# ImIntheMiddle/VATL4Pose-WACV2024

Hardware: AMD Instinct MI355X
Metric: frames/sec pose-infer+uncertainty, 256x192 17-kp (higher is better)
Workload: dtype f32; 1 GPU; SimpleBaseline-R50 256x192 inference + decode + local-peak + THC-L1, 1024-frame synthetic video per GPU; frames_per_gpu=1024, batch=1024, tracks=4, parallelism=frame-sharded x1

## Files before the change

include/vatl_hip.h:

```cpp
#ifndef VATL_HIP_H
#define VATL_HIP_H

#include <stdint.h>

#ifdef __cplusplus
extern "C" {
#endif

#define VATL_VERSION 100
#define VATL_EINVAL  (-1)
#define VATL_ELAUNCH (-2)

int         vatl_version(void);
const char* vatl_last_error(void);

int vatl_flop_meter_begin(void);
int vatl_flop_meter_end(double* direct_flops, double* winograd_flops, int64_t* direct_launches, int64_t* winograd_launches);
#define VATL_ROUTE_NAMES "igemm,igemm_bnbwd,igemm_dma,persistent_1x1,streamk,rows_1x1,bottleneck_chain,stem_pool,halo_3x3," \
                         "winograd,winograd_2h,winograd_bnbwd,winograd_persist,winograd_c32,wgrad,winograd_wgrad,winograd_wgrad_2h," \
                         "winograd_wgrad_table,winograd_f4,winograd_f4_bnbwd,gemm1x1_ring,winograd_deconv43,winograd_s2_43,stem_pool_w1d," \
                         "chain_proj,chain_step"
int vatl_flop_meter_routes(int64_t* counts, int n);


int vatl_nchw_to_nhwc(const float* src, float* dst, int N, int C, int H, int W, int Cpad, void* stream);
int vatl_nhwc_to_nchw(const float* src, float* dst, int N, int C, int H, int W, void* stream);

int vatl_pack_conv_weight(const float* w_oihw, float* w_packed, int Cout, int Cin, int R, int S,
                          int CoutPad, int Spad, int CinPad, void* stream);
int vatl_pack_deconv4x4s2_weight(const float* w_iohw, float* w_packed, int Cin, int Cout, int CoutPad, void* stream);
int64_t vatl_stem_pool_weight_floats(void);
int vatl_pack_stem_pool_weight(const float* w_oihw, float* packed, void* stream);
int vatl_stem_pool_supported(int H, int W);
int vatl_stem7x7s2_pool_fwd(const float* x_nchw, const float* w_packed, const float* scale, const float* bias, float* y_nhwc,
                            int N, int H, int W, void* stream);
int64_t vatl_stem_pool_w1d_weight_floats(void);
int vatl_pack_stem_pool_w1d_weight(const float* w_oihw, float* packed, void* stream);
int vatl_stem_pool_w1d_supported(int H, int W);
int vatl_stem7x7s2_pool_w1d_fwd(const float* x_nchw, const float* w_packed, const float* scale, const float* bias, float* y_nhwc,
                                int N, int H, int W, void* stream);
int64_t vatl_stem3_weight_floats(void);
int vatl_pack_stem3_weight(const float* w_oihw, float* packed, void* stream);
int vatl_stem3x3s2_fwd(const float* x_nchw, const float* w_packed, const float* scale, const float* bias, float* y_nhwc,
                       int N, int H, int W, void* stream);

// ... 19 lines not shown
                                 int Cin, int Cout, int relu, void* stream);
int64_t vatl_winograd_f4_stats_row_blocks(int64_t N, int H, int W);
int vatl_conv3x3_winograd_f4_fwd_stats(const float* x, const float* u, float* y, double* stats, int64_t* row_blocks_used, int N, int H, int W, int Cin, int Cout,
                                       void* stream);
int vatl_conv3x3_winograd_f4_fwd_bnbwd(const float* x, const float* u, const float* residual, float* y, int N, int H, int W, int Cin, int Cout, const float* bn_z,
                                       const float* bn_mask_y, const float* bn_scale, const float* bn_bias, const float* bn_mean, const float* bn_invstd,
                                       double* stats, int64_t* row_blocks_used, void* stream);

int vatl_conv1x1_rows_supported(int K1, int K2, int N, int64_t M);
int vatl_conv1x1_rows_fwd(const float* a, const float* x2, const float* w, const float* scale, const float* bias, const float* residual, float* y,
                          int64_t M, int K1, int K2, int N, int relu, void* stream);

int vatl_bottleneck_chain_supported(int Cmid, int Cout, int Cnext, int64_t M);
int vatl_bottleneck_chain_fwd(const float* a, const float* w3, const float* scale3, const float* bias3, const float* skip, float* t,
                              const float* w1, const float* scale1, const float* bias1, float* y1, int64_t M, int Cmid, int Cout,
                              int Cnext, void* stream);

int vatl_chain_proj_supported(int Cmid, int Cout, int Cnext, int64_t M);
int vatl_chain_proj_fwd(const float* a, const float* x2, const float* w, const float* scale, const float* bias, float* t, const float* w1,
                        const float* scale1, const float* bias1, float* y1, int64_t M, int Cmid, int Cout, int Cnext, int relu, void* stream);
int vatl_chain_step_supported(int Cmid, int Cout, int Cnext, int64_t M);
int vatl_chain_step_fwd(const float* a, const float* w3, const float* scale3, const float* bias3, const float* skip, float* t, const float* w1,
                        const float* scale1, const float* bias1, float* y1, int64_t M, int Cmid, int Cout, int Cnext, void* stream);

int vatl_tune_set(int knob, int value);
int vatl_set_splitk_workspace(float* workspace, int64_t floats);
int vatl_set_splitk_workspace_thread(float* workspace, int64_t floats);
int64_t vatl_streamk_workspace_bytes(void);
int vatl_set_streamk_workspace_thread(void* workspace, int64_t bytes);
int vatl_conv_cout_pad(int Cout);
int vatl_conv2d_fwd(const float* x, const float* w, const float* scale, const float* bias, const float* residual,
                    float* y, int N, int H, int W, int Cin, int Cout, int CoutPad, int R, int S, int stride, int pad,
                    int relu, int out_nchw, void* stream);

int vatl_deconv4x4s2_fwd(const float* x, const float* w, const float* scale, const float* bias, float* y,
                         int N, int H, int W, int Cin, int Cout, int CoutPad, int relu, void* stream);

int vatl_maxpool3x3s2_fwd(const float* x, float* y, int N, int H, int W, int C, void* stream);
int vatl_gap_fwd(const float* x, float* y, int N, int HW, int C, void* stream);

int vatl_pixelshuffle2_fwd(const float* x, float* y, int N, int H, int W, int C, void* stream);
int vatl_se_scale_add_relu(const float* x, const float* gate, const float* residual, float* y, int N, int HW, int C, void* stream);
int vatl_fuse_upsample_add(const float* base, const float* z0, int shift0, const float* z1, int shift1, const float* z2, int shift2,
                           float* y, int N, int H, int W, int C, int relu, void* stream);
int vatl_upsample_nearest_bwd(const float* dy, const float* yact_or_null, float* dz, int N, int H, int W, int C, int shift, void* stream);
int vatl_gap_bwd(const float* dy, float* dx, int N, int HW, int C, void* stream);
// ... 215 lines not shown
```

vatl4pose-wacv2024_amd/alphapose/models/hip_engine.py:

```python
from __future__ import annotations

import time
import weakref

import torch
import torch.nn as nn

import vatl_hip as vh

MAX_CHUNK = 1024



WINOGRAD = True
ROWS_GEMM = True
ROWS_GEMM_K = (128, 256)
WINO_C32 = True
WINO_F4 = True
DECONV_43 = True
S2_43 = True


class _Conv:
    __slots__ = ("w", "u", "u32", "u4", "us2", "wsrc", "wino", "c32", "f4", "s2", "scale", "bias", "cout", "r", "s", "stride", "pad")
# ... 66 lines not shown
        return vh.deconv4x4s2_fwd(x, self.w, self.scale, self.bias, self.cout, relu)


def _d(p):
    return None if p is None else p.detach()


FUSE_PROJ = True


class _BottleneckPlan:
    def __init__(self, blk):
        self.c1 = _Conv(blk.conv1, blk.bn1)
        self.c2 = _Conv(blk.conv2, blk.bn2)
        self.c3 = _Conv(blk.conv3, blk.bn3)
        self.proj = _Conv(blk.downsample[0], blk.downsample[1]) if blk.downsample is not None else None
        self.dual = None
        if (FUSE_PROJ and self.proj is not None and type(self) is _BottleneckPlan and self.proj.r == 1 and self.c3.cout >= 128
                and blk.conv3.in_channels % 32 == 0 and blk.downsample[0].in_channels % 32 == 0):
            w, b = vh.pack_conv1x1_dual_weight(blk.conv3.weight.detach(), self.c3.scale, self.c3.bias, blk.downsample[0].weight.detach(),
                                               self.proj.scale, self.proj.bias)
            self.dual = (w, b, self.proj.stride)

    def __call__(self, x, out=None, y1=None, nxt=None):
        y = y1 if y1 is not None else self.c1(x, relu=True)
        y = self.c2(y, relu=True)
        return self.tail(y, x, out=out, nxt=nxt)

    def tail(self, y, x, out=None, nxt=None):
        if self.dual is not None:
            if (ROWS_GEMM and self.dual[2] == 1 and y.shape[-1] == 64 and x.shape[-1] == 64 and not vh.latency_mode()
                    and vh.conv1x1_rows_supported(64, 64, self.c3.cout, y.shape[0] * y.shape[1] * y.shape[2])):
                if nxt is not None and FUSE_CHAIN_PROJ and vh.chain_proj_supported(64, self.c3.cout, nxt[0].shape[0], y.shape[0] * y.shape[1] * y.shape[2]):
                    return vh.conv1x1_rows_fwd(y, self.dual[0], None, self.dual[1], self.c3.cout, True, x2=x, out=out, next_conv1=nxt)
                t = vh.conv1x1_rows_fwd(y, self.dual[0], None, self.dual[1], self.c3.cout, True, x2=x, out=out)
            else:
                t = vh.conv1x1_dual_fwd(y, x, self.dual[0], self.dual[1], self.c3.cout, self.dual[2], True, out=out)
        else:
            skip = x if self.proj is None else self.proj(x, relu=False)
            t = self.c3(y, relu=True, residual=skip, out=out)
        return t if nxt is None else (t, None)


FUSE_CHAIN = True
FUSE_CHAIN_PROJ = True
FUSE_CHAIN_STEP = True


def _conv1_of(nxt, cout):
    if (type(nxt) is _BottleneckPlan and (nxt.c1.r, nxt.c1.stride, nxt.c1.pad) == (1, 1, 0) and nxt.c1.scale is not None and nxt.c1.cout == cout
            and not vh.latency_mode()):
        return nxt.c1.w, nxt.c1.scale, nxt.c1.bias
    return None


def _run_blocks(blocks, x, out=None):
    y1 = None
    for k, b in enumerate(blocks):
        last = k == len(blocks) - 1
        o = out if last else None
        if type(b) is not _BottleneckPlan:
            x, y1 = b(x), None
            continue
        nxt = None if last else blocks[k + 1]
        m = x.shape[0] * x.shape[1] * x.shape[2]
        chain = (FUSE_CHAIN and b.proj is None and not vh.latency_mode() and b.c3.scale is not None
                 and vh.bottleneck_chain_supported(b.c3.w.shape[-1], b.c3.cout, 0, m))
        if not chain:
            c1 = _conv1_of(nxt, 64) if b.dual is not None and FUSE_CHAIN_PROJ else None
            x, y1 = b(x, out=o, y1=y1, nxt=c1) if c1 is not None else (b(x, out=o, y1=y1), None)
            continue
        y = b.c2(y1 if y1 is not None else b.c1(x, relu=True), relu=True)
        link, step = _conv1_of(nxt, 64), _conv1_of(nxt, 128) if FUSE_CHAIN_STEP else None
        if link is not None and vh.bottleneck_chain_supported(b.c3.w.shape[-1], b.c3.cout, 64, m):
            x, y1 = vh.bottleneck_chain_fwd(y, b.c3.w, b.c3.scale, b.c3.bias, x, *link, out=o)
        elif step is not None and vh.chain_step_supported(b.c3.w.shape[-1], b.c3.cout, 128, m):
            x, y1 = vh.bottleneck_chain_fwd(y, b.c3.w, b.c3.scale, b.c3.bias, x, out=o, next_stage_conv1=step)
        else:
            x, y1 = vh.bottleneck_chain_fwd(y, b.c3.w, b.c3.scale, b.c3.bias, x, out=o)[0], None
    return x


FUSE_STEM = True
STEM_W1D = True


def _stem_pool_weight(net):
    c = net.conv1
    ok = (FUSE_STEM and tuple(c.weight.shape) == (64, 3, 7, 7) and c.stride == (2, 2) and c.padding == (3, 3) and c.bias is None
          and isinstance(net.maxpool, nn.MaxPool2d) and net.maxpool.kernel_size in (3, (3, 3)) and net.maxpool.stride in (2, (2, 2))
          and net.maxpool.padding in (1, (1, 1)) and not net.maxpool.ceil_mode)
    return vh.pack_stem_pool_weight(c.weight.detach()) if ok else None


class _TrunkPlan:
    def __init__(self, net):
        self.stem = _Conv(net.conv1, net.bn1)
        self.stem_pw = _stem_pool_weight(net)
        self.stem_src, self.stem_u1d = net.conv1.weight.detach(), None
        self.blocks = [_BottleneckPlan(b) for stage in net.stages() for b in stage]
# ... 408 lines not shown
```

vatl4pose-wacv2024_amd/csrc/bottleneck_chain.hip:

```cpp
#include "common.h"
#include "buffer.h"

namespace vatl {

struct ChainParams {
    const float* a;
    const float* w3;
    const float* scale3;
    const float* bias3;
    const float* res;
    float* t;
    const float* w1;
    const float* scale1;
    const float* bias1;
    float* out2;
    int M, N2, relu3;
    int m_tiles;
    unsigned a_bytes, t_bytes, o_bytes, w3_bytes, w1_bytes;
};

constexpr unsigned BOOB = 0xFFFFFFFFu;

constexpr int BT_LDT = 260;
constexpr int BT_AS = 32 * 64;
// ... 137 lines not shown
                    buf_store4(orr, ((unsigned)(mt * 32 + row) * 64u + (unsigned)q4 * 4u) * 4u, o);
                }
            }
        }
        if constexpr (SECOND) asm volatile("s_waitcnt vmcnt(10)" ::: "memory");
        else asm volatile("s_waitcnt vmcnt(8)" ::: "memory");
    }
}


struct FormParams {
    const float* a;
    const float* x2;
    const float* w3;
    const float* scale3;
    const float* bias3;
    const float* res;
    float* t;
    const float* w1;
    const float* scale1;
    const float* bias1;
    float* y;
    int m_tiles, relu3;
    unsigned a_bytes, t_bytes, y_bytes;
};

__device__ __forceinline__ unsigned uadd(unsigned s_part, unsigned v_part) {
#if defined(__HIP_DEVICE_COMPILE__)
    unsigned r;
    asm("v_add_u32 %0, %1, %2" : "=v"(r) : "s"(s_part), "v"(v_part));
    return r;
#else
    return s_part + v_part;
#endif
}

constexpr int CF_TS = 4 * 32 * 64;

template <bool PROJ>
__global__ __launch_bounds__(256, 2) void chain_form_kernel(FormParams p) {
    constexpr int K1 = PROJ ? 128 : 64, G1 = K1 / 8, AS = 32 * K1, N2 = PROJ ? 64 : 128;
    extern __shared__ __attribute__((aligned(16))) float smem[];
    float* As = smem;
    float* Ts = smem + 2 * AS;
    const int tid = threadIdx.x, lane = tid & 63, wave = __builtin_amdgcn_readfirstlane(tid >> 6);
    const int fr = lane & 31, h = lane >> 5;
    const int nblk = gridDim.x;

    const __amdgpu_buffer_rsrc_t ar = buf_rsrc(p.a, p.a_bytes);
    const __amdgpu_buffer_rsrc_t xr = buf_rsrc(PROJ ? p.x2 : p.a, PROJ ? p.a_bytes : 0u);
    const __amdgpu_buffer_rsrc_t w3r = buf_rsrc(p.w3, 256u * K1 * 4u);
    const __amdgpu_buffer_rsrc_t w1r = buf_rsrc(p.w1, (unsigned)N2 * 256u * 4u);
    const __amdgpu_buffer_rsrc_t tr = buf_rsrc(p.t, p.t_bytes);
    const __amdgpu_buffer_rsrc_t rr = buf_rsrc(p.res ? p.res : p.t, p.res ? p.t_bytes : 0u);
    const __amdgpu_buffer_rsrc_t yr = buf_rsrc(p.y, p.y_bytes);

    f32x4 w3f[2][G1];
#pragma unroll
    for (int nb = 0; nb < 2; ++nb)
#pragma unroll
        for (int g = 0; g < G1; ++g) w3f[nb][g] = buf_load4(w3r, (unsigned)(((wave * 64 + nb * 32 + fr) * K1 + 8 * g + 4 * h) * 4));
    float sc3[2], bi3[2];
#pragma unroll
    for (int nb = 0; nb < 2; ++nb) {
        const int n = wave * 64 + nb * 32 + fr;
        sc3[nb] = p.scale3 ? p.scale3[n] : 1.f;
        bi3[nb] = p.bias3 ? p.bias3[n] : 0.f;
    }
    const int l16 = lane & 15, j = lane >> 4;
    const int n1 = PROJ ? wave * 16 + l16 : wave * 32 + fr;
    f32x4 w1f[PROJ ? 16 : 32];
#pragma unroll
    for (int g = 0; g < (PROJ ? 16 : 32); ++g) w1f[g] = buf_load4(w1r, (unsigned)((n1 * 256 + (PROJ ? 16 * g + 4 * j : 8 * g + 4 * h)) * 4));
    const float sc1 = p.scale1 ? p.scale1[n1] : 1.f, bi1 = p.bias1 ? p.bias1[n1] : 0.f;
    const float lo3 = p.relu3 ? 0.f : -INFINITY;

    const int c4 = lane, r0 = wave;
// ... 47 lines not shown
        __builtin_amdgcn_sched_barrier(0);
        const int abase = buf * AS, tqbase = wave * 2048;
#pragma unroll
        for (int nb = 0; nb < 2; ++nb) {
            f32x16 acc;
#pragma unroll
            for (int e = 0; e < 16; ++e) acc[e] = 0.f;
#pragma unroll
            for (int g = 0; g < G1; ++g) {
                const f32x4 af = *reinterpret_cast<const f32x4*>(smem + abase + ax[g & 3] + 32 * (g >> 2));
#pragma unroll
                for (int tt = 0; tt < 4; ++tt) acc = __builtin_amdgcn_mfma_f32_32x32x2f32(af[tt], w3f[nb][g][tt], acc, 0, 0, 0);
            }
            if (!PROJ && nb == 0) asm volatile("s_waitcnt vmcnt(2)" ::: "memory");
#pragma unroll
            for (int e = 0; e < 16; ++e) {
                float* q = smem + tqbase + tq[e & 3] + 64 * ((e & 3) + 8 * (e >> 2)) + 32 * nb;
                const float v = acc[e] * sc3[nb] + bi3[nb];
                *q = fmaxf(v + (PROJ ? 0.f : *q), lo3);
            }
        }
        lds_barrier();
#pragma unroll
        for (int u = 0; u < 8; ++u)
            buf_store4(tr, uadd((unsigned)mt * (32u * 1024u) + (unsigned)(r0 + 4 * u) * 1024u, (unsigned)c4 * 16u),
                       *reinterpret_cast<const f32x4*>(smem + r0 * 64 + tw[u & 1] + 256 * u));
        const unsigned ytile = (unsigned)mt * (32u * N2 * 4u) + (unsigned)wave * (PROJ ? 64u : 128u);
        if constexpr (PROJ) {
            f32x4 acc2[2] = {f32x4{0.f, 0.f, 0.f, 0.f}, f32x4{0.f, 0.f, 0.f, 0.f}};
#pragma unroll
            for (int q = 0; q < 16; ++q) {
                f32x4 tf[2];
#pragma unroll
                for (int rb = 0; rb < 2; ++rb) tf[rb] = *reinterpret_cast<const f32x4*>(smem + tx[q & 1] + 32 * ((q >> 1) & 1) + 2048 * (q >> 2) + 1024 * rb);
#pragma unroll
                for (int tt = 0; tt < 4; ++tt)
#pragma unroll
                    for (int rb = 0; rb < 2; ++rb) acc2[rb] = __builtin_amdgcn_mfma_f32_16x16x4f32(tf[rb][tt], w1f[q][tt], acc2[rb], 0, 0, 0);
            }
#pragma unroll
            for (int rb = 0; rb < 2; ++rb)
#pragma unroll
                for (int r = 0; r < 4; ++r) buf_store1(yr, uadd(ytile + (unsigned)(rb * 16 + r) * (N2 * 4u), vy), fmaxf(acc2[rb][r] * sc1 + bi1, 0.f));
            asm volatile("s_waitcnt vmcnt(16)" ::: "memory");
        } else {
            f32x16 acc2;
#pragma unroll
            for (int e = 0; e < 16; ++e) acc2[e] = 0.f;
#pragma unroll
// ... 35 lines not shown
        if (int rc = ensure_dynamic_lds(reinterpret_cast<const void*>(kern), smem, c1, "bottleneck_chain")) return rc;
        const int grid = p.m_tiles < 512 ? p.m_tiles : 512;
        hipLaunchKernelGGL(kern, dim3(grid), dim3(256), smem, (hipStream_t)stream, p);
        meter_add(0, 2.0 * padded * 256.0 * 64.0 * 2.0);
        meter_route(kRouteChain);
    } else {
        auto kern = bottleneck_chain_kernel<false>;
        if (int rc = ensure_dynamic_lds(reinterpret_cast<const void*>(kern), smem, c0, "bottleneck_chain")) return rc;
        const int grid = p.m_tiles < 512 ? p.m_tiles : 512;
        hipLaunchKernelGGL(kern, dim3(grid), dim3(256), smem, (hipStream_t)stream, p);
        meter_add(0, 2.0 * padded * 256.0 * 64.0);
        meter_route(kRouteChain);
    }
    return check_launch("bottleneck_chain");
}

static bool form_shape_ok(int Cmid, int Cout, int Cnext, int want_next, int64_t M) {
    return Cmid == 64 && Cout == 256 && Cnext == want_next && M > 0 && (M + 32) * 256 < (1LL << 30);
}

extern "C" int vatl_chain_proj_supported(int Cmid, int Cout, int Cnext, int64_t M) { return form_shape_ok(Cmid, Cout, Cnext, 64, M) ? 1 : 0; }
extern "C" int vatl_chain_step_supported(int Cmid, int Cout, int Cnext, int64_t M) { return form_shape_ok(Cmid, Cout, Cnext, 128, M) ? 1 : 0; }

static int chain_form_launch(bool proj, FormParams p, int64_t M, void* stream) {
    const int N2 = proj ? 64 : 128, K1 = proj ? 128 : 64;
    const char* what = proj ? "chain_proj" : "chain_step";
    p.m_tiles = (int)((M + 31) / 32);
    p.a_bytes = (unsigned)(M * 64 * 4); p.t_bytes = (unsigned)(M * 256 * 4); p.y_bytes = (unsigned)(M * N2 * 4);
    const int smem = (2 * 32 * K1 + CF_TS) * (int)sizeof(float);
    static std::atomic<unsigned> c[2] = {{0}, {0}};
    void (*kern)(FormParams) = chain_form_kernel<false>;
    if (proj) kern = chain_form_kernel<true>;
    if (int rc = ensure_dynamic_lds(reinterpret_cast<const void*>(kern), smem, c[proj], what)) return rc;
    const int grid = p.m_tiles < 512 ? p.m_tiles : 512;
    hipLaunchKernelGGL(kern, dim3(grid), dim3(256), smem, (hipStream_t)stream, p);
    meter_add(0, 2.0 * ((double)p.m_tiles * 32.0) * 256.0 * (double)(K1 + N2));
    meter_route(proj ? kRouteChainProj : kRouteChainStep);
    return check_launch(what);
}

extern "C" int vatl_chain_proj_fwd(const float* a, const float* x2, const float* w, const float* scale, const float* bias, float* t, const float* w1, const float* scale1,
                                   const float* bias1, float* y1, int64_t M, int Cmid, int Cout, int Cnext, int relu, void* stream) {
    if (!a || !x2 || !w || !t || !w1 || !y1) return fail(VATL_EINVAL, "chain_proj_fwd: bad arguments");
    if (!form_shape_ok(Cmid, Cout, Cnext, 64, M)) return fail(VATL_EINVAL, "chain_proj_fwd: serves 64 + 64 -> 256 -> 64 channels and (M + 32) * 256 < 2^30 pixels x channels");
    FormParams p{};
    p.a = a; p.x2 = x2; p.w3 = w; p.scale3 = scale; p.bias3 = bias; p.t = t; p.w1 = w1; p.scale1 = scale1; p.bias1 = bias1; p.y = y1; p.relu3 = relu;
    return chain_form_launch(true, p, M, stream);
}

extern "C" int vatl_chain_step_fwd(const float* a, const float* w3, const float* scale3, const float* bias3, const float* skip, float* t, const float* w1,
                                   const float* scale1, const float* bias1, float* y1, int64_t M, int Cmid, int Cout, int Cnext, void* stream) {
    if (!a || !w3 || !t || !w1 || !y1) return fail(VATL_EINVAL, "chain_step_fwd: bad arguments");
    if (!form_shape_ok(Cmid, Cout, Cnext, 128, M)) return fail(VATL_EINVAL, "chain_step_fwd: serves 64 -> 256 -> 128 channels and (M + 32) * 256 < 2^30 pixels x channels");
    FormParams p{};
    p.a = a; p.w3 = w3; p.scale3 = scale3; p.bias3 = bias3; p.res = skip; p.t = t; p.w1 = w1; p.scale1 = scale1; p.bias1 = bias1; p.y = y1; p.relu3 = 1;
    return chain_form_launch(false, p, M, stream);
}
```

vatl4pose-wacv2024_amd/csrc/common.h:

```cpp
#pragma once
#include <hip/hip_runtime.h>
#include <atomic>
#include <cstdarg>
#include <cstdio>
#include <cstdint>

#include "vatl_hip.h"

namespace vatl {

char* err_buf();
int fail(int code, const char* fmt, ...);

void meter_add(int kind, double flops);
enum MeterRoute {
    kRouteIgemm = 0, kRouteIgemmBnBwd, kRouteIgemmDma, kRoutePersistent1x1, kRouteStreamK, kRouteRows, kRouteChain, kRouteStemPool, kRouteHalo,
    kRouteWino, kRouteWino2H, kRouteWinoBnBwd, kRouteWinoPersist, kRouteWinoC32, kRouteWgrad, kRouteWinoWgrad, kRouteWinoWgrad2H,
    kRouteWinoWgradTable, kRouteWinoF4, kRouteWinoF4BnBwd, kRouteGemm1x1Ring, kRouteWinoDeconv43, kRouteWinoS2_43, kRouteStemPoolW1d, kRouteChainProj,
    kRouteChainStep, kRouteCount
};
void meter_route(int route);

inline int check_launch(const char* what) {
    hipError_t e = hipGetLastError();
    if (e != hipSuccess) return fail(VATL_ELAUNCH, "%s: %s", what, hipGetErrorString(e));
    return 0;
}

inline int ensure_dynamic_lds(const void* kern, int bytes, std::atomic<unsigned>& done_mask, const char* what) {
    int d = 0;
    if (hipGetDevice(&d) != hipSuccess) return fail(VATL_ELAUNCH, "%s: no current device", what);
    const unsigned bit = 1u << (d & 31);
    if (done_mask.load(std::memory_order_acquire) & bit) return 0;
    hipError_t e = hipFuncSetAttribute(kern, hipFuncAttributeMaxDynamicSharedMemorySize, bytes);
    if (e != hipSuccess) return fail(VATL_ELAUNCH, "hipFuncSetAttribute(%s): %s", what, hipGetErrorString(e));
    done_mask.fetch_or(bit, std::memory_order_release);
    return 0;
}

__attribute__((visibility("hidden"))) int conv3x3_halo_try(const float* x, const float* w, const float* scale, const float* bias, const float* residual, float* y, int N, int H, int W,
                                                           int Cin, int Cout, int CoutPad, int R, int S, int stride, int pad, int relu, hipStream_t st);

static inline int cdiv(int64_t a, int64_t b) { return (int)((a + b - 1) / b); }

// ... 49 lines not shown
```

vatl4pose-wacv2024_amd/csrc/runtime.hip:

```cpp
#include "common.h"

namespace vatl {

static thread_local char g_err[512] = "";
char* err_buf() { return g_err; }
int fail(int code, const char* fmt, ...) {
    va_list ap;
    va_start(ap, fmt);
    vsnprintf(g_err, sizeof(g_err), fmt, ap);
    va_end(ap);
    return code;
}

static thread_local bool tl_meter_on = false;
static thread_local double tl_meter_flops[2] = {0.0, 0.0};
static thread_local long long tl_meter_launches[2] = {0, 0};
void meter_add(int kind, double flops) {
    if (!tl_meter_on) return;
    tl_meter_flops[kind & 1] += flops;
    tl_meter_launches[kind & 1] += 1;
}
static thread_local long long tl_meter_routes[kRouteCount] = {};
void meter_route(int route) {
    if (tl_meter_on && route >= 0 && route < kRouteCount) tl_meter_routes[route] += 1;
}
void meter_begin() {
    tl_meter_on = true; tl_meter_flops[0] = tl_meter_flops[1] = 0.0; tl_meter_launches[0] = tl_meter_launches[1] = 0;
    for (int k = 0; k < kRouteCount; ++k) tl_meter_routes[k] = 0;
}
int meter_routes(long long* out, int n) {
    for (int k = 0; k < n && k < kRouteCount; ++k) out[k] = tl_meter_routes[k];
    return kRouteCount;
}
void meter_end(double* flops, long long* launches) {
    for (int k = 0; k < 2; ++k) { flops[k] = tl_meter_flops[k]; launches[k] = tl_meter_launches[k]; }
    tl_meter_on = false;
}

}

using namespace vatl;

extern "C" int vatl_version(void) { return VATL_VERSION; }
extern "C" const char* vatl_last_error(void) { return err_buf(); }

extern "C" int vatl_flop_meter_begin(void) { vatl::meter_begin(); return 0; }
extern "C" int vatl_flop_meter_end(double* direct_flops, double* winograd_flops, int64_t* direct_launches, int64_t* winograd_launches) {
    double f[2]; long long n[2];
    vatl::meter_end(f, n);
    if (direct_flops) *direct_flops = f[0];
    if (winograd_flops) *winograd_flops = f[1];
    if (direct_launches) *direct_launches = n[0];
    if (winograd_launches) *winograd_launches = n[1];
    return 0;
}
extern "C" int vatl_flop_meter_routes(int64_t* counts, int n) {
    if (!counts || n < 0) return vatl::fail(VATL_EINVAL, "flop_meter_routes: null pointer");
    long long tmp[64] = {};
    const int have = vatl::meter_routes(tmp, n < 64 ? n : 64);
    for (int k = 0; k < n; ++k) counts[k] = k < have && k < 64 ? (int64_t)tmp[k] : 0;
    return have;
}
```

vatl4pose-wacv2024_amd/vatl_hip/__init__.py:

```python
from __future__ import annotations

import ctypes as C
import os
import threading as _threading

import torch

_HERE = os.path.dirname(os.path.abspath(__file__))
LIB_PATH = os.environ.get("VATL_HIP_LIB") or os.path.join(_HERE, "libvatl_hip.so")

_p = C.c_void_p
_i = C.c_int
_f = C.c_float
_d = C.c_double
_i64 = C.c_int64

SIGNATURES = {
    "vatl_version": (_i, []),
    "vatl_last_error": (C.c_char_p, []),
    "vatl_flop_meter_begin": (_i, []),
    "vatl_flop_meter_end": (_i, [_p, _p, _p, _p]),
    "vatl_flop_meter_routes": (_i, [_p, _i]),
    "vatl_nchw_to_nhwc": (_i, [_p, _p, _i, _i, _i, _i, _i, _p]),
    "vatl_nhwc_to_nchw": (_i, [_p, _p, _i, _i, _i, _i, _p]),
    "vatl_pack_conv_weight": (_i, [_p, _p, _i, _i, _i, _i, _i, _i, _i, _p]),
    "vatl_pack_deconv4x4s2_weight": (_i, [_p, _p, _i, _i, _i, _p]),
    "vatl_pack_conv1x1_dual_weight": (_i, [_p, _p, _p, _p, _p, _p, _p, _p, _i, _i, _i, _i, _p]),
    "vatl_conv1x1_dual_fwd": (_i, [_p, _p, _p, _p, _p, _i, _i, _i, _i, _i, _i, _i, _i, _i, _i, _i, _p]),
    "vatl_winograd_c32_weight_floats": (_i64, []),
    "vatl_pack_winograd_c32_weight": (_i, [_p, _p, _p]),
    "vatl_conv3x3_winograd_c32_supported": (_i, [_i, _i, _i, _i, _i]),
    "vatl_conv3x3_winograd_c32_fwd": (_i, [_p, _p, _p, _p, _p, _p, _i, _i, _i, _i, _p]),
    "vatl_winograd_f4_weight_floats": (_i64, [_i, _i]),
    "vatl_pack_winograd_f4_weight": (_i, [_p, _p, _i, _i, _i, _p]),
    "vatl_winograd_f4_stats_row_blocks": (_i64, [_i64, _i, _i]),
    "vatl_conv3x3_winograd_f4_fwd_stats": (_i, [_p, _p, _p, _p, _p, _i, _i, _i, _i, _i, _p]),
    "vatl_conv3x3_winograd_f4_fwd_bnbwd": (_i, [_p, _p, _p, _p, _i, _i, _i, _i, _i, _p, _p, _p, _p, _p, _p, _p, _p, _p]),
    "vatl_conv3x3_winograd_f4_supported": (_i, [_i, _i, _i, _i, _i]),
    "vatl_conv3x3_winograd_f4_fwd": (_i, [_p, _p, _p, _p, _p, _p, _i, _i, _i, _i, _i, _i, _p]),
    "vatl_conv1x1_rows_supported": (_i, [_i, _i, _i, _i64]),
    "vatl_conv1x1_rows_fwd": (_i, [_p, _p, _p, _p, _p, _p, _p, _i64, _i, _i, _i, _i, _p]),
    "vatl_bottleneck_chain_supported": (_i, [_i, _i, _i, _i64]),
    "vatl_bottleneck_chain_fwd": (_i, [_p, _p, _p, _p, _p, _p, _p, _p, _p, _p, _i64, _i, _i, _i, _p]),
    "vatl_chain_proj_supported": (_i, [_i, _i, _i, _i64]),
    "vatl_chain_proj_fwd": (_i, [_p, _p, _p, _p, _p, _p, _p, _p, _p, _p, _i64, _i, _i, _i, _i, _p]),
    "vatl_chain_step_supported": (_i, [_i, _i, _i, _i64]),
    "vatl_chain_step_fwd": (_i, [_p, _p, _p, _p, _p, _p, _p, _p, _p, _p, _i64, _i, _i, _i, _p]),
    "vatl_stem_pool_weight_floats": (_i64, []),
    "vatl_pack_stem_pool_weight": (_i, [_p, _p, _p]),
    "vatl_stem_pool_supported": (_i, [_i, _i]),
    "vatl_stem_pool_w1d_weight_floats": (_i64, []),
    "vatl_pack_stem_pool_w1d_weight": (_i, [_p, _p, _p]),
    "vatl_stem_pool_w1d_supported": (_i, [_i, _i]),
    "vatl_stem7x7s2_pool_w1d_fwd": (_i, [_p] * 5 + [_i] * 3 + [_p]),
    "vatl_stem7x7s2_pool_fwd": (_i, [_p, _p, _p, _p, _p, _i, _i, _i, _p]),
    "vatl_stem3_weight_floats": (_i64, []),
    "vatl_pack_stem3_weight": (_i, [_p, _p, _p]),
    "vatl_stem3x3s2_fwd": (_i, [_p, _p, _p, _p, _p, _i, _i, _i, _p]),
    "vatl_bn_fold": (_i, [_p, _p, _p, _p, _p, _f, _p, _p, _i, _p]),
    "vatl_tune_set": (_i, [_i, _i]),
    "vatl_set_splitk_workspace": (_i, [_p, _i64]),
    "vatl_set_splitk_workspace_thread": (_i, [_p, _i64]),
    "vatl_streamk_workspace_bytes": (_i64, []),
    "vatl_set_streamk_workspace_thread": (_i, [_p, _i64]),
    "vatl_conv_cout_pad": (_i, [_i]),
    "vatl_conv2d_fwd": (_i, [_p, _p, _p, _p, _p, _p, _i, _i, _i, _i, _i, _i, _i, _i, _i, _i, _i, _i, _p]),
    "vatl_deconv4x4s2_fwd": (_i, [_p, _p, _p, _p, _p, _i, _i, _i, _i, _i, _i, _i, _p]),
    "vatl_maxpool3x3s2_fwd": (_i, [_p, _p, _i, _i, _i, _i, _p]),
    "vatl_gap_fwd": (_i, [_p, _p, _i, _i, _i, _p]),
    "vatl_pixelshuffle2_fwd": (_i, [_p, _p, _i, _i, _i, _i, _p]),
# ... 164 lines not shown
_tls = _threading.local()



def nchw_to_nhwc(x: torch.Tensor, cpad: int | None = None) -> torch.Tensor:
    n, c, h, w = x.shape
    cpad = cpad or c
    y = torch.empty((n, h, w, cpad), device=x.device, dtype=torch.float32)
    _check(lib().vatl_nchw_to_nhwc(_ptr(x), _ptr(y), n, c, h, w, cpad, _stream()), "vatl_nchw_to_nhwc")
    return y


def nhwc_to_nchw(x: torch.Tensor) -> torch.Tensor:
    n, h, w, c = x.shape
    y = torch.empty((n, c, h, w), device=x.device, dtype=torch.float32)
    _check(lib().vatl_nhwc_to_nchw(_ptr(x), _ptr(y), n, c, h, w, _stream()), "vatl_nhwc_to_nchw")
    return y



ROUTE_NAMES = ("igemm", "igemm_bnbwd", "igemm_dma", "persistent_1x1", "streamk", "rows_1x1", "bottleneck_chain", "stem_pool", "halo_3x3", "winograd",
               "winograd_2h", "winograd_bnbwd", "winograd_persist", "winograd_c32", "wgrad", "winograd_wgrad", "winograd_wgrad_2h", "winograd_wgrad_table", "winograd_f4", "winograd_f4_bnbwd",
               "gemm1x1_ring", "winograd_deconv43", "winograd_s2_43", "stem_pool_w1d", "chain_proj", "chain_step")


class flop_meter:

    def __enter__(self):
        _check(lib().vatl_flop_meter_begin(), "flop_meter_begin")
        self.direct = self.winograd = self.total = 0.0
        self.direct_launches = self.winograd_launches = 0
        return self

    @staticmethod
    def launches_now() -> int:
        counts = (C.c_int64 * len(ROUTE_NAMES))()
        _check(min(0, lib().vatl_flop_meter_routes(counts, len(ROUTE_NAMES))), "flop_meter_routes")
        return int(sum(counts))

    def __exit__(self, *exc):
        counts = (C.c_int64 * len(ROUTE_NAMES))()
        _check(min(0, lib().vatl_flop_meter_routes(counts, len(ROUTE_NAMES))), "flop_meter_routes")
        self.routes = {n: int(c) for n, c in zip(ROUTE_NAMES, counts)}
        d, w, nd, nw = C.c_double(0), C.c_double(0), C.c_int64(0), C.c_int64(0)
        _check(lib().vatl_flop_meter_end(C.byref(d), C.byref(w), C.byref(nd), C.byref(nw)), "flop_meter_end")
        self.direct, self.winograd, self.total = d.value, w.value, d.value + w.value
        self.direct_launches, self.winograd_launches = nd.value, nw.value
        return False


def tune_set(knob: int, value: int):
    _check(lib().vatl_tune_set(knob, value), "vatl_tune_set")


_splitk_buf = {}


def enable_splitk(megabytes: int = 64, device=None):
    dev = torch.device(device) if device is not None else torch.device("cuda", torch.cuda.current_device())
    idx = dev.index if dev.index is not None else torch.cuda.current_device()
    with torch.cuda.device(idx):
        if megabytes <= 0:
            _check(lib().vatl_set_splitk_workspace(None, 0), "vatl_set_splitk_workspace")
            _splitk_buf.pop(idx, None)
            return
        buf = torch.empty(megabytes * (1 << 18), device=torch.device("cuda", idx), dtype=torch.float32)
# ... 369 lines not shown
        assert w1.numel() == cnext * cout
        y1 = y1_out if y1_out is not None else torch.empty((n, h, w_, cnext), device=a.device, dtype=torch.float32)
        assert y1.is_contiguous()
        _check(lib().vatl_chain_proj_fwd(_ptr(a), _ptr(x2), _ptr(w), _ptr(scale), _ptr(bias), _ptr(y), _ptr(w1), _ptr(scale1), _ptr(bias1), _ptr(y1),
                                         n * h * w_, k1, cout, cnext, int(relu), _stream()), "vatl_chain_proj_fwd")
        return y, y1
    _check(lib().vatl_conv1x1_rows_fwd(_ptr(a), _ptr(x2), _ptr(w), _ptr(scale), _ptr(bias), _ptr(residual), _ptr(y), n * h * w_, k1, k2, cout, int(relu),
                                       _stream()), "vatl_conv1x1_rows_fwd")
    return y


def bottleneck_chain_supported(cmid: int, cout: int, cnext: int, m: int) -> bool:
    return bool(lib().vatl_bottleneck_chain_supported(cmid, cout, cnext, m))


def chain_proj_supported(cmid: int, cout: int, cnext: int, m: int) -> bool:
    return bool(lib().vatl_chain_proj_supported(cmid, cout, cnext, m))


def chain_step_supported(cmid: int, cout: int, cnext: int, m: int) -> bool:
    return bool(lib().vatl_chain_step_supported(cmid, cout, cnext, m))


def bottleneck_chain_fwd(a, w3, scale3, bias3, skip, w1=None, scale1=None, bias1=None, out=None, y1_out=None, next_stage_conv1=None):
    n, h, w_, cmid = a.shape
    cout = w3.shape[0]
    step = next_stage_conv1 is not None
    if step:
        if w1 is not None:
            raise VatlError("bottleneck_chain_fwd: w1 and next_stage_conv1 are exclusive")
        w1, scale1, bias1 = next_stage_conv1
    cnext = 0 if w1 is None else w1.shape[0]
    assert w3.numel() == cout * cmid and (w1 is None or w1.numel() == cnext * cout) and (skip is None or tuple(skip.shape) == (n, h, w_, cout))
    t = out if out is not None else torch.empty((n, h, w_, cout), device=a.device, dtype=torch.float32)
    assert t.is_contiguous() and a.is_contiguous() and (skip is None or skip.is_contiguous())
    y1 = None if w1 is None else (y1_out if y1_out is not None else torch.empty((n, h, w_, cnext), device=a.device, dtype=torch.float32))
    assert y1 is None or y1.is_contiguous()
    fn, name = (lib().vatl_chain_step_fwd, "vatl_chain_step_fwd") if step else (lib().vatl_bottleneck_chain_fwd, "vatl_bottleneck_chain_fwd")
    _check(fn(_ptr(a), _ptr(w3), _ptr(scale3), _ptr(bias3), _ptr(skip), _ptr(t), _ptr(w1), _ptr(scale1), _ptr(bias1), _ptr(y1),
              n * h * w_, cmid, cout, cnext, _stream()), name)
    return t, y1


def stem3_fwd(x_nchw: torch.Tensor, w_packed: torch.Tensor, scale: torch.Tensor, bias: torch.Tensor, out=None) -> torch.Tensor:
    n, c, h, w = x_nchw.shape
    if c != 3:
        raise VatlError(f"stem3_fwd: expected 3 input channels, got {c}")
    y = out if out is not None else torch.empty((n, h // 2, w // 2, 64), device=x_nchw.device, dtype=torch.float32)
    _check(lib().vatl_stem3x3s2_fwd(_ptr(x_nchw), _ptr(w_packed), _ptr(scale), _ptr(bias), _ptr(y), n, h, w, _stream()), "vatl_stem3x3s2_fwd")
    return y


def stem_pool_supported(h: int, w: int) -> bool:
    return bool(lib().vatl_stem_pool_supported(int(h), int(w)))


def stem_pool_w1d_supported(h: int, w: int) -> bool:
    return bool(lib().vatl_stem_pool_w1d_supported(int(h), int(w)))


# ... 847 lines not shown
```

Measured before the change: 17660 frames/s.

## Store only stride-2 subsampled block output in chain-step kernel for projection consumer

When the last layer1 bottleneck feeds a stage whose stride-2 1x1 projection only reads even pixels, the fused chain-step kernel now writes just the subsampled residual output t. Odd-position rows are sent to an out-of-range buffer offset so the stores are dropped. The next block's dual conv then runs with stride 1 on the compact tensor. This removes three quarters of the t writes and gives the projection a dense read, at the cost of per-row fast-division index math and a new kernel variant. A variant counter is added to the meter.

Measured after the change: 17730 frames/s (median of 6 runs). No clear change (+0.4%).

```diff
diff --git a/include/vatl_hip.h b/include/vatl_hip.h
--- a/include/vatl_hip.h
+++ b/include/vatl_hip.h
@@ -21,6 +21,8 @@
                          "winograd_wgrad_table,winograd_f4,winograd_f4_bnbwd,gemm1x1_ring,winograd_deconv43,winograd_s2_43,stem_pool_w1d," \
                          "chain_proj,chain_step"
 int vatl_flop_meter_routes(int64_t* counts, int n);
+#define VATL_VARIANT_NAMES "chain_step_sub"
+int vatl_flop_meter_variants(int64_t* counts, int n);
 
 
 int vatl_nchw_to_nhwc(const float* src, float* dst, int N, int C, int H, int W, int Cpad, void* stream);
@@ -86,6 +88,9 @@
 int vatl_chain_step_supported(int Cmid, int Cout, int Cnext, int64_t M);
 int vatl_chain_step_fwd(const float* a, const float* w3, const float* scale3, const float* bias3, const float* skip, float* t, const float* w1,
                         const float* scale1, const float* bias1, float* y1, int64_t M, int Cmid, int Cout, int Cnext, void* stream);
+int vatl_chain_step_sub_supported(int Cmid, int Cout, int Cnext, int N, int H, int W);
+int vatl_chain_step_sub_fwd(const float* a, const float* w3, const float* scale3, const float* bias3, const float* skip, float* t_sub, const float* w1,
+                            const float* scale1, const float* bias1, float* y1, int N, int H, int W, int Cmid, int Cout, int Cnext, void* stream);
 
 int vatl_tune_set(int knob, int value);
 int vatl_set_splitk_workspace(float* workspace, int64_t floats);
diff --git a/vatl4pose-wacv2024_amd/alphapose/models/hip_engine.py b/vatl4pose-wacv2024_amd/alphapose/models/hip_engine.py
--- a/vatl4pose-wacv2024_amd/alphapose/models/hip_engine.py
+++ b/vatl4pose-wacv2024_amd/alphapose/models/hip_engine.py
@@ -112,12 +112,20 @@
                                                self.proj.scale, self.proj.bias)
             self.dual = (w, b, self.proj.stride)
 
-    def __call__(self, x, out=None, y1=None, nxt=None):
+    def __call__(self, x, out=None, y1=None, nxt=None, x_sub=False):
+        assert y1 is not None or not x_sub
         y = y1 if y1 is not None else self.c1(x, relu=True)
         y = self.c2(y, relu=True)
-        return self.tail(y, x, out=out, nxt=nxt)
-
-    def tail(self, y, x, out=None, nxt=None):
+        return self.tail(y, x, out=out, nxt=nxt, x_sub=x_sub)
+
+    def takes_subsampled_input(self):
+        return self.dual is not None and self.dual[2] == 2 and (self.proj.r, self.proj.pad) == (1, 0)
+
+    def tail(self, y, x, out=None, nxt=None, x_sub=False):
+        if x_sub:
+            assert self.takes_subsampled_input() and tuple(x.shape[:3]) == tuple(y.shape[:3])
+            t = vh.conv1x1_dual_fwd(y, x, self.dual[0], self.dual[1], self.c3.cout, 1, True, out=out)
+            return t if nxt is None else (t, None)
         if self.dual is not None:
             if (ROWS_GEMM and self.dual[2] == 1 and y.shape[-1] == 64 and x.shape[-1] == 64 and not vh.latency_mode()
                     and vh.conv1x1_rows_supported(64, 64, self.c3.cout, y.shape[0] * y.shape[1] * y.shape[2])):
@@ -135,6 +143,7 @@
 FUSE_CHAIN = True
 FUSE_CHAIN_PROJ = True
 FUSE_CHAIN_STEP = True
+FUSE_CHAIN_STEP_SUB = True
 
 
 def _conv1_of(nxt, cout):
@@ -145,7 +154,7 @@
 
 
 def _run_blocks(blocks, x, out=None):
-    y1 = None
+    y1, x_sub = None, False
     for k, b in enumerate(blocks):
         last = k == len(blocks) - 1
         o = out if last else None
@@ -157,6 +166,9 @@
         chain = (FUSE_CHAIN and b.proj is None and not vh.latency_mode() and b.c3.scale is not None
                  and vh.bottleneck_chain_supported(b.c3.w.shape[-1], b.c3.cout, 0, m))
         if not chain:
+            if x_sub:
+                x, y1, x_sub = b(x, out=o, y1=y1, x_sub=True), None, False
+                continue
             c1 = _conv1_of(nxt, 64) if b.dual is not None and FUSE_CHAIN_PROJ else None
             x, y1 = b(x, out=o, y1=y1, nxt=c1) if c1 is not None else (b(x, out=o, y1=y1), None)
             continue
@@ -165,7 +177,9 @@
         if link is not None and vh.bottleneck_chain_supported(b.c3.w.shape[-1], b.c3.cout, 64, m):
             x, y1 = vh.bottleneck_chain_fwd(y, b.c3.w, b.c3.scale, b.c3.bias, x, *link, out=o)
         elif step is not None and vh.chain_step_supported(b.c3.w.shape[-1], b.c3.cout, 128, m):
-            x, y1 = vh.bottleneck_chain_fwd(y, b.c3.w, b.c3.scale, b.c3.bias, x, out=o, next_stage_conv1=step)
+            x_sub = (FUSE_CHAIN_STEP_SUB and o is None and nxt.takes_subsampled_input()
+                     and vh.chain_step_sub_supported(b.c3.w.shape[-1], b.c3.cout, 128, x.shape[0], x.shape[1], x.shape[2]))
+            x, y1 = vh.bottleneck_chain_fwd(y, b.c3.w, b.c3.scale, b.c3.bias, x, out=o, next_stage_conv1=step, t_subsampled=x_sub)
         else:
             x, y1 = vh.bottleneck_chain_fwd(y, b.c3.w, b.c3.scale, b.c3.bias, x, out=o)[0], None
     return x
diff --git a/vatl4pose-wacv2024_amd/csrc/bottleneck_chain.hip b/vatl4pose-wacv2024_amd/csrc/bottleneck_chain.hip
--- a/vatl4pose-wacv2024_amd/csrc/bottleneck_chain.hip
+++ b/vatl4pose-wacv2024_amd/csrc/bottleneck_chain.hip
@@ -183,7 +183,9 @@
     const float* bias1;
     float* y;
     int m_tiles, relu3;
-    unsigned a_bytes, t_bytes, y_bytes;
+    unsigned a_bytes, t_bytes, y_bytes, r_bytes;
+    int hw, w, hw2, w2;
+    FastDivU d_hw, d_w;
 };
 
 __device__ __forceinline__ unsigned uadd(unsigned s_part, unsigned v_part) {
@@ -198,8 +200,9 @@
 
 constexpr int CF_TS = 4 * 32 * 64;
 
-template <bool PROJ>
+template <bool PROJ, bool SUB = false>
 __global__ __launch_bounds__(256, 2) void chain_form_kernel(FormParams p) {
+    static_assert(!(PROJ && SUB), "the sub-sampled store belongs to form S");
     constexpr int K1 = PROJ ? 128 : 64, G1 = K1 / 8, AS = 32 * K1, N2 = PROJ ? 64 : 128;
     extern __shared__ __attribute__((aligned(16))) float smem[];
     float* As = smem;
@@ -213,7 +216,7 @@
     const __amdgpu_buffer_rsrc_t w3r = buf_rsrc(p.w3, 256u * K1 * 4u);
     const __amdgpu_buffer_rsrc_t w1r = buf_rsrc(p.w1, (unsigned)N2 * 256u * 4u);
     const __amdgpu_buffer_rsrc_t tr = buf_rsrc(p.t, p.t_bytes);
-    const __amdgpu_buffer_rsrc_t rr = buf_rsrc(p.res ? p.res : p.t, p.res ? p.t_bytes : 0u);
+    const __amdgpu_buffer_rsrc_t rr = buf_rsrc(p.res ? p.res : p.t, p.res ? p.r_bytes : 0u);
     const __amdgpu_buffer_rsrc_t yr = buf_rsrc(p.y, p.y_bytes);
 
     f32x4 w3f[2][G1];
@@ -307,9 +310,16 @@
         }
         lds_barrier();
 #pragma unroll
-        for (int u = 0; u < 8; ++u)
-            buf_store4(tr, uadd((unsigned)mt * (32u * 1024u) + (unsigned)(r0 + 4 * u) * 1024u, (unsigned)c4 * 16u),
-                       *reinterpret_cast<const f32x4*>(smem + r0 * 64 + tw[u & 1] + 256 * u));
+        for (int u = 0; u < 8; ++u) {
+            unsigned trow = (unsigned)mt * (32u * 1024u) + (unsigned)(r0 + 4 * u) * 1024u;
+            if constexpr (SUB) {
+                const int m = mt * 32 + r0 + 4 * u;
+                const int img = fdiv(m, p.d_hw), rem = m - img * p.hw;
+                const int y = fdiv(rem, p.d_w), x = rem - y * p.w;
+                trow = ((y | x) & 1) ? 0x80000000u : (unsigned)(img * p.hw2 + (y >> 1) * p.w2 + (x >> 1)) * 1024u;
+            }
+            buf_store4(tr, uadd(trow, (unsigned)c4 * 16u), *reinterpret_cast<const f32x4*>(smem + r0 * 64 + tw[u & 1] + 256 * u));
+        }
         const unsigned ytile = (unsigned)mt * (32u * N2 * 4u) + (unsigned)wave * (PROJ ? 64u : 128u);
         if constexpr (PROJ) {
             f32x4 acc2[2] = {f32x4{0.f, 0.f, 0.f, 0.f}, f32x4{0.f, 0.f, 0.f, 0.f}};
@@ -391,20 +401,28 @@
 extern "C" int vatl_chain_proj_supported(int Cmid, int Cout, int Cnext, int64_t M) { return form_shape_ok(Cmid, Cout, Cnext, 64, M) ? 1 : 0; }
 extern "C" int vatl_chain_step_supported(int Cmid, int Cout, int Cnext, int64_t M) { return form_shape_ok(Cmid, Cout, Cnext, 128, M) ? 1 : 0; }
 
-static int chain_form_launch(bool proj, FormParams p, int64_t M, void* stream) {
+static int chain_form_launch(bool proj, FormParams p, int64_t M, void* stream, int sub_h = 0, int sub_w = 0) {
     const int N2 = proj ? 64 : 128, K1 = proj ? 128 : 64;
-    const char* what = proj ? "chain_proj" : "chain_step";
+    const bool sub = sub_h > 0;
+    const char* what = proj ? "chain_proj" : sub ? "chain_step_sub" : "chain_step";
     p.m_tiles = (int)((M + 31) / 32);
-    p.a_bytes = (unsigned)(M * 64 * 4); p.t_bytes = (unsigned)(M * 256 * 4); p.y_bytes = (unsigned)(M * N2 * 4);
+    p.a_bytes = (unsigned)(M * 64 * 4); p.t_bytes = p.r_bytes = (unsigned)(M * 256 * 4); p.y_bytes = (unsigned)(M * N2 * 4);
+    if (sub) {
+        p.hw = sub_h * sub_w; p.w = sub_w; p.hw2 = p.hw / 4; p.w2 = sub_w / 2;
+        p.d_hw = make_fastdiv((unsigned)p.hw); p.d_w = make_fastdiv((unsigned)p.w);
+        p.t_bytes = (unsigned)(M / 4 * 256 * 4);
+    }
     const int smem = (2 * 32 * K1 + CF_TS) * (int)sizeof(float);
-    static std::atomic<unsigned> c[2] = {{0}, {0}};
+    static std::atomic<unsigned> c[3] = {{0}, {0}, {0}};
     void (*kern)(FormParams) = chain_form_kernel<false>;
     if (proj) kern = chain_form_kernel<true>;
-    if (int rc = ensure_dynamic_lds(reinterpret_cast<const void*>(kern), smem, c[proj], what)) return rc;
+    if (sub) kern = chain_form_kernel<false, true>;
+    if (int rc = ensure_dynamic_lds(reinterpret_cast<const void*>(kern), smem, c[sub ? 2 : proj], what)) return rc;
     const int grid = p.m_tiles < 512 ? p.m_tiles : 512;
     hipLaunchKernelGGL(kern, dim3(grid), dim3(256), smem, (hipStream_t)stream, p);
     meter_add(0, 2.0 * ((double)p.m_tiles * 32.0) * 256.0 * (double)(K1 + N2));
     meter_route(proj ? kRouteChainProj : kRouteChainStep);
+    if (sub) meter_variant(kVariantChainStepSub);
     return check_launch(what);
 }
 
@@ -425,3 +443,19 @@
     p.a = a; p.w3 = w3; p.scale3 = scale3; p.bias3 = bias3; p.res = skip; p.t = t; p.w1 = w1; p.scale1 = scale1; p.bias1 = bias1; p.y = y1; p.relu3 = 1;
     return chain_form_launch(false, p, M, stream);
 }
+
+static bool step_sub_ok(int Cmid, int Cout, int Cnext, int N, int H, int W) {
+    return N > 0 && H > 0 && W > 0 && !(H & 1) && !(W & 1) && form_shape_ok(Cmid, Cout, Cnext, 128, (int64_t)N * H * W);
+}
+
+extern "C" int vatl_chain_step_sub_supported(int Cmid, int Cout, int Cnext, int N, int H, int W) { return step_sub_ok(Cmid, Cout, Cnext, N, H, W) ? 1 : 0; }
+
+extern "C" int vatl_chain_step_sub_fwd(const float* a, const float* w3, const float* scale3, const float* bias3, const float* skip, float* t_sub, const float* w1,
+                                       const float* scale1, const float* bias1, float* y1, int N, int H, int W, int Cmid, int Cout, int Cnext, void* stream) {
+    if (!a || !w3 || !t_sub || !w1 || !y1) return fail(VATL_EINVAL, "chain_step_sub_fwd: bad arguments");
+    if (!step_sub_ok(Cmid, Cout, Cnext, N, H, W))
+        return fail(VATL_EINVAL, "chain_step_sub_fwd: serves 64 -> 256 -> 128 channels, even H and W and (N H W + 32) * 256 < 2^30 pixels x channels");
+    FormParams p{};
+    p.a = a; p.w3 = w3; p.scale3 = scale3; p.bias3 = bias3; p.res = skip; p.t = t_sub; p.w1 = w1; p.scale1 = scale1; p.bias1 = bias1; p.y = y1; p.relu3 = 1;
+    return chain_form_launch(false, p, (int64_t)N * H * W, stream, H, W);
+}
diff --git a/vatl4pose-wacv2024_amd/csrc/common.h b/vatl4pose-wacv2024_amd/csrc/common.h
--- a/vatl4pose-wacv2024_amd/csrc/common.h
+++ b/vatl4pose-wacv2024_amd/csrc/common.h
@@ -20,6 +20,8 @@
     kRouteChainStep, kRouteCount
 };
 void meter_route(int route);
+enum MeterVariant { kVariantChainStepSub = 0, kVariantCount };
+void meter_variant(int variant);
 
 inline int check_launch(const char* what) {
     hipError_t e = hipGetLastError();
diff --git a/vatl4pose-wacv2024_amd/csrc/runtime.hip b/vatl4pose-wacv2024_amd/csrc/runtime.hip
--- a/vatl4pose-wacv2024_amd/csrc/runtime.hip
+++ b/vatl4pose-wacv2024_amd/csrc/runtime.hip
@@ -24,9 +24,18 @@
 void meter_route(int route) {
     if (tl_meter_on && route >= 0 && route < kRouteCount) tl_meter_routes[route] += 1;
 }
+static thread_local long long tl_meter_variants[kVariantCount] = {};
+void meter_variant(int variant) {
+    if (tl_meter_on && variant >= 0 && variant < kVariantCount) tl_meter_variants[variant] += 1;
+}
 void meter_begin() {
     tl_meter_on = true; tl_meter_flops[0] = tl_meter_flops[1] = 0.0; tl_meter_launches[0] = tl_meter_launches[1] = 0;
     for (int k = 0; k < kRouteCount; ++k) tl_meter_routes[k] = 0;
+    for (int k = 0; k < kVariantCount; ++k) tl_meter_variants[k] = 0;
+}
+int meter_variants(long long* out, int n) {
+    for (int k = 0; k < n && k < kVariantCount; ++k) out[k] = tl_meter_variants[k];
+    return kVariantCount;
 }
 int meter_routes(long long* out, int n) {
     for (int k = 0; k < n && k < kRouteCount; ++k) out[k] = tl_meter_routes[k];
@@ -61,3 +70,10 @@
     for (int k = 0; k < n; ++k) counts[k] = k < have && k < 64 ? (int64_t)tmp[k] : 0;
     return have;
 }
+extern "C" int vatl_flop_meter_variants(int64_t* counts, int n) {
+    if (!counts || n < 0) return vatl::fail(VATL_EINVAL, "flop_meter_variants: null pointer");
+    long long tmp[16] = {};
+    const int have = vatl::meter_variants(tmp, n < 16 ? n : 16);
+    for (int k = 0; k < n; ++k) counts[k] = k < have && k < 16 ? (int64_t)tmp[k] : 0;
+    return have;
+}
diff --git a/vatl4pose-wacv2024_amd/vatl_hip/__init__.py b/vatl4pose-wacv2024_amd/vatl_hip/__init__.py
--- a/vatl4pose-wacv2024_amd/vatl_hip/__init__.py
+++ b/vatl4pose-wacv2024_amd/vatl_hip/__init__.py
@@ -21,6 +21,7 @@
     "vatl_flop_meter_begin": (_i, []),
     "vatl_flop_meter_end": (_i, [_p, _p, _p, _p]),
     "vatl_flop_meter_routes": (_i, [_p, _i]),
+    "vatl_flop_meter_variants": (_i, [_p, _i]),
     "vatl_nchw_to_nhwc": (_i, [_p, _p, _i, _i, _i, _i, _i, _p]),
     "vatl_nhwc_to_nchw": (_i, [_p, _p, _i, _i, _i, _i, _p]),
     "vatl_pack_conv_weight": (_i, [_p, _p, _i, _i, _i, _i, _i, _i, _i, _p]),
@@ -46,6 +47,8 @@
     "vatl_chain_proj_fwd": (_i, [_p, _p, _p, _p, _p, _p, _p, _p, _p, _p, _i64, _i, _i, _i, _i, _p]),
     "vatl_chain_step_supported": (_i, [_i, _i, _i, _i64]),
     "vatl_chain_step_fwd": (_i, [_p, _p, _p, _p, _p, _p, _p, _p, _p, _p, _i64, _i, _i, _i, _p]),
+    "vatl_chain_step_sub_supported": (_i, [_i, _i, _i, _i, _i, _i]),
+    "vatl_chain_step_sub_fwd": (_i, [_p, _p, _p, _p, _p, _p, _p, _p, _p, _p, _i, _i, _i, _i, _i, _i, _p]),
     "vatl_stem_pool_weight_floats": (_i64, []),
     "vatl_pack_stem_pool_weight": (_i, [_p, _p, _p]),
     "vatl_stem_pool_supported": (_i, [_i, _i]),
@@ -256,6 +259,7 @@
 ROUTE_NAMES = ("igemm", "igemm_bnbwd", "igemm_dma", "persistent_1x1", "streamk", "rows_1x1", "bottleneck_chain", "stem_pool", "halo_3x3", "winograd",
                "winograd_2h", "winograd_bnbwd", "winograd_persist", "winograd_c32", "wgrad", "winograd_wgrad", "winograd_wgrad_2h", "winograd_wgrad_table", "winograd_f4", "winograd_f4_bnbwd",
                "gemm1x1_ring", "winograd_deconv43", "winograd_s2_43", "stem_pool_w1d", "chain_proj", "chain_step")
+VARIANT_NAMES = ("chain_step_sub",)
 
 
 class flop_meter:
@@ -276,6 +280,9 @@
         counts = (C.c_int64 * len(ROUTE_NAMES))()
         _check(min(0, lib().vatl_flop_meter_routes(counts, len(ROUTE_NAMES))), "flop_meter_routes")
         self.routes = {n: int(c) for n, c in zip(ROUTE_NAMES, counts)}
+        counts = (C.c_int64 * len(VARIANT_NAMES))()
+        _check(min(0, lib().vatl_flop_meter_variants(counts, len(VARIANT_NAMES))), "flop_meter_variants")
+        self.variants = {n: int(c) for n, c in zip(VARIANT_NAMES, counts)}
         d, w, nd, nw = C.c_double(0), C.c_double(0), C.c_int64(0), C.c_int64(0)
         _check(lib().vatl_flop_meter_end(C.byref(d), C.byref(w), C.byref(nd), C.byref(nw)), "flop_meter_end")
         self.direct, self.winograd, self.total = d.value, w.value, d.value + w.value
@@ -691,7 +698,11 @@
     return bool(lib().vatl_chain_step_supported(cmid, cout, cnext, m))
 
 
-def bottleneck_chain_fwd(a, w3, scale3, bias3, skip, w1=None, scale1=None, bias1=None, out=None, y1_out=None, next_stage_conv1=None):
+def chain_step_sub_supported(cmid: int, cout: int, cnext: int, n: int, h: int, w: int) -> bool:
+    return bool(lib().vatl_chain_step_sub_supported(cmid, cout, cnext, n, h, w))
+
+
+def bottleneck_chain_fwd(a, w3, scale3, bias3, skip, w1=None, scale1=None, bias1=None, out=None, y1_out=None, next_stage_conv1=None, t_subsampled=False):
     n, h, w_, cmid = a.shape
     cout = w3.shape[0]
     step = next_stage_conv1 is not None
@@ -699,12 +710,19 @@
         if w1 is not None:
             raise VatlError("bottleneck_chain_fwd: w1 and next_stage_conv1 are exclusive")
         w1, scale1, bias1 = next_stage_conv1
+    elif t_subsampled:
+        raise VatlError("bottleneck_chain_fwd: t_subsampled goes with next_stage_conv1")
     cnext = 0 if w1 is None else w1.shape[0]
     assert w3.numel() == cout * cmid and (w1 is None or w1.numel() == cnext * cout) and (skip is None or tuple(skip.shape) == (n, h, w_, cout))
-    t = out if out is not None else torch.empty((n, h, w_, cout), device=a.device, dtype=torch.float32)
-    assert t.is_contiguous() and a.is_contiguous() and (skip is None or skip.is_contiguous())
+    t_shape = (n, h // 2, w_ // 2, cout) if t_subsampled else (n, h, w_, cout)
+    t = out if out is not None else torch.empty(t_shape, device=a.device, dtype=torch.float32)
+    assert tuple(t.shape) == t_shape and t.is_contiguous() and a.is_contiguous() and (skip is None or skip.is_contiguous())
     y1 = None if w1 is None else (y1_out if y1_out is not None else torch.empty((n, h, w_, cnext), device=a.device, dtype=torch.float32))
     assert y1 is None or y1.is_contiguous()
+    if t_subsampled:
+        _check(lib().vatl_chain_step_sub_fwd(_ptr(a), _ptr(w3), _ptr(scale3), _ptr(bias3), _ptr(skip), _ptr(t), _ptr(w1), _ptr(scale1), _ptr(bias1), _ptr(y1),
+                                             n, h, w_, cmid, cout, cnext, _stream()), "vatl_chain_step_sub_fwd")
+        return t, y1
     fn, name = (lib().vatl_chain_step_fwd, "vatl_chain_step_fwd") if step else (lib().vatl_bottleneck_chain_fwd, "vatl_bottleneck_chain_fwd")
     _check(fn(_ptr(a), _ptr(w3), _ptr(scale3), _ptr(bias3), _ptr(skip), _ptr(t), _ptr(w1), _ptr(scale1), _ptr(bias1), _ptr(y1),
               n * h * w_, cmid, cout, cnext, _stream()), name)
```
